# jp-schneider/awesome

Measured on AMD Instinct MI355X. Metric: INR-fits/sec (256x256 grid, convexity prior), higher is better.
Workload: dtype f32; 1 GPU; 1 x 256x256 synthetic convex blob per GPU, ConvexNextNet(h=130,L=1), SE(sigmoid) mean, Adam lr 2e-3, clamp, E=2000 full-batch steps (BASELINE configs[1]); images_per_gpu=1, grid=256x256, epochs_per_fit=2000, parallelism=dp1 (independent fits)

## Files before the change

awesome_amd/csrc/icnn_step2.h:

```cpp
#pragma once
#include "icnn_step.h"


namespace {

template <int H, int C>
struct Cfg2 {
    using G1 = Cfg<H, C>;
    static constexpr int TM = G1::TM, HM = G1::HM, HR = G1::HR, NEXT = G1::NEXT, NRL = G1::NRL, KG = G1::KG, PT = G1::PT;
    static constexpr int S = G1::S, SA = G1::SA, SB = G1::SB, RPW = G1::RPW;
    static constexpr int ext_pos(int e) { return G1::ext_pos(e); }
    static constexpr int nr_in(int tk) { return G1::nr_in(tk); }
    static constexpr int OFF_SC = 0;
    static constexpr int OFF_WINE = OFF_SC + 8;
    static constexpr int OFF_WIN = OFF_WINE + 4 * PT;
    static constexpr int OFF_BIN = OFF_WIN + C * 16;
    static constexpr int OFF_FLOOR = OFF_BIN + 16;
    static constexpr int OFF_WO = OFF_FLOOR + 16;
    static constexpr int OFF_WCT0 = OFF_WO + PT;
    static constexpr int OFF_WCT1 = OFF_WCT0 + HR * PT;
    static constexpr int WREG = round_up(H * S + 16, 256);
    static constexpr int OFF_W0 = round_up(OFF_WCT1 + HR * PT, 4);
    static constexpr int OFF_W1 = OFF_W0 + WREG;
    static constexpr int IMG_FLOATS = OFF_W1 + WREG;
    static constexpr int STAGE_FLOATS = SP * SA + 16 + SP * SB + 16;
    static constexpr bool ALIAS = STAGE_FLOATS <= WREG;
    static constexpr int OFF_STA = ALIAS ? OFF_W1 : IMG_FLOATS;
    static constexpr int OFF_STB = OFF_STA + SP * SA + 16;
    static constexpr int OFF_ACC = ALIAS ? IMG_FLOATS : IMG_FLOATS + STAGE_FLOATS;
    static constexpr int LDS_FLOATS = OFF_ACC + 4 * PT;
    static constexpr int LDS_BYTES = LDS_FLOATS * 4;
    static_assert(LDS_BYTES <= 160 * 1024, "LDS budget exceeded");
    static_assert(OFF_W0 % 4 == 0 && IMG_FLOATS % 4 == 0, "alignment");
    static constexpr int P_WIN = 0;
    static constexpr int P_BIN = H * C;
    static constexpr int P_W1 = P_BIN + H;
    static constexpr int P_B1 = P_W1 + H * H;
// ... 52 lines not shown
        constexpr int NV4 = G::IMG_FLOATS / 4;
        for (int i0 = 0; i0 < NV4; i0 += 8 * WG_THREADS) {
            f32x4 tmp[8];
#pragma unroll
            for (int k = 0; k < 8; ++k) {
                const int i = i0 + tid + k * WG_THREADS;
                if (i < NV4) tmp[k] = src[i];
            }
#pragma unroll
            for (int k = 0; k < 8; ++k) {
                const int i = i0 + tid + k * WG_THREADS;
                if (i < NV4) ((f32x4*)smem)[i] = tmp[k];
            }
        }
    }
    float cfg_ = 0.f, cbg_ = 0.f;
    if (TRAIN) {
        cfg_ = a.coef[2 * img];
        cbg_ = a.coef[2 * img + 1];
        for (int i = tid; i < 4 * PT; i += WG_THREADS) accW[i] = 0.f;
    }
    __syncthreads();
    const float b_o = smem[G::OFF_SC];
    float s_o[C];
#pragma unroll
    for (int c = 0; c < C; ++c) s_o[c] = smem[G::OFF_SC + 1 + c];
    float wol[HRA];
#pragma unroll
    for (int u = 0; u < HRA; ++u) wol[u] = HR > 0 ? woT[HM + u] : 0.f;
    const bool row_ok = wave * RPW < TM;
    const int arow = 16 * wave * RPW + l15;

    f32x4 dWa[RPW][KG], dWb[RPW][KG];
    f32x4 dL0[TM];
    float dwol[HRA], dWla[HRA][KG], dWlb[HRA][KG], dL0l[HRA][NEXT];
    float loss_acc = 0.f, dbo = 0.f, dso[C];
    if (TRAIN) {
#pragma unroll
        for (int j = 0; j < RPW; ++j)
#pragma unroll
            for (int b = 0; b < KG; ++b) {
                dWa[j][b] = f32x4{0.f, 0.f, 0.f, 0.f};
                dWb[j][b] = f32x4{0.f, 0.f, 0.f, 0.f};
            }
#pragma unroll
        for (int t = 0; t < TM; ++t) dL0[t] = f32x4{0.f, 0.f, 0.f, 0.f};
#pragma unroll
        for (int u = 0; u < HRA; ++u) {
            dwol[u] = 0.f;
#pragma unroll
            for (int b = 0; b < KG; ++b) {
                dWla[u][b] = 0.f;
                dWlb[u][b] = 0.f;
            }
#pragma unroll
            for (int e = 0; e < NEXT; ++e) dL0l[u][e] = 0.f;
        }
#pragma unroll
        for (int c = 0; c < C; ++c) dso[c] = 0.f;
    }

    auto gemm_fwd = [&](const float* Wl, const f32x4 (&B)[KG], f32x4 (&acc)[TM], float (&la)[HRA]) {
        const float* const wf = Wl + l15 * S + 4 * g;
#pragma unroll
        for (int u = 0; u < HRA; ++u) la[u] = 0.f;
        f32x4 wq[2][TM], wlq[2][HRA];
#pragma unroll
        for (int t = 0; t < TM; ++t) wq[0][t] = *(const f32x4*)(wf + t * 16 * S);
#pragma unroll
        for (int u = 0; u < HR; ++u) wlq[0][u] = *(const f32x4*)(Wl + (HM + u) * S + 4 * g);
#pragma unroll
        for (int tk = 0; tk < KG; ++tk) {
            const int cur = tk & 1, nx = cur ^ 1;
            auto next_read = [&](int i) {
                if (tk + 1 < KG) {
                    if (i < TM) wq[nx][i] = *(const f32x4*)(wf + i * 16 * S + 16 * (tk + 1));
                    else wlq[nx][i - TM] = *(const f32x4*)(Wl + (HM + i - TM) * S + 16 * (tk + 1) + 4 * g);
                }
            };
            constexpr int NRD = TM + HR;
            const int nmf = G::nr_in(tk) * TM;
            const int every = nmf / NRD > 0 ? nmf / NRD : 1;
#pragma unroll
            for (int r = 0; r < G::nr_in(tk); ++r) {
#pragma unroll
                for (int t = 0; t < TM; ++t) {
                    acc[t] = MFMA16(wq[cur][t][r], B[tk][r], (tk == 0 && r == 0) ? (f32x4{0.f, 0.f, 0.f, 0.f}) : acc[t]);
                    const int q = r * TM + t;
                    if (q % every == every - 1 && q / every < NRD) next_read(q / every);
                    OPERAND_FENCE();
                }
            }
#pragma unroll
            for (int i = 0; i < NRD; ++i)
                if (i >= nmf / every) next_read(i);
#pragma unroll
            for (int u = 0; u < HR; ++u)
#pragma unroll
                for (int r = 0; r < G::nr_in(tk); ++r) la[u] = fmaf(wlq[cur][u][r], B[tk][r], la[u]);
            __builtin_amdgcn_sched_barrier(0);
        }
    };
    auto gemm_bwd = [&](auto swap_tag, const float* Wl, const float* WcTl, const f32x4 (&dz)[TM], const float (&dzl)[HRA],
                        f32x4 (&out)[TM], float (&outl)[HRA], f32x4& outx) {
        constexpr bool SWAP = decltype(swap_tag)::value;
        float bqx[2] = {0.f, 0.f};
        outx = f32x4{0.f, 0.f, 0.f, 0.f};
        constexpr int KS = 4 * TM + HR;
        const float* const wb = Wl + l15;
#pragma unroll
        for (int u = 0; u < HRA; ++u) outl[u] = 0.f;
        float bq[2][TM];
        f32x4 wcq[2][HRA];
        auto b_row = [&](int ks) -> const float* {
            const int tk = ks >> 2, r = ks & 3;
            if (tk < TM) return wb + (16 * tk + 4 * g + r) * S;
            return wb + (g == 0 ? (HM + r) * S : 0);
        };
        {
            const float* br = b_row(0);
#pragma unroll
            for (int t = 0; t < TM; ++t) bq[0][t] = br[16 * t];
            if (DX) bqx[0] = br[16 * TM];
#pragma unroll
            for (int u = 0; u < HR; ++u) wcq[0][u] = *(const f32x4*)(WcTl + u * PT + 4 * g);
        }
#pragma unroll
        for (int ks = 0; ks < KS; ++ks) {
            const int tk = ks >> 2, r = ks & 3;
            if (ks + 1 < KS) {
                const float* br = b_row(ks + 1);
                if (DX) bqx[(ks + 1) & 1] = br[16 * TM];
            }
            if (r == 0 && (tk + 1) * 4 < KS) {
#pragma unroll
                for (int u = 0; u < HR; ++u) wcq[(tk + 1) & 1][u] = *(const f32x4*)(WcTl + u * PT + 16 * (tk + 1) + 4 * g);
            }
            OPERAND_FENCE();
            const float bop = tk < TM ? dz[tk < TM ? tk : 0][r] : (g == 0 ? dzl[r < HRA ? r : 0] : 0.f);
#pragma unroll
            for (int t = 0; t < TM; ++t) {
                const f32x4 c0 = ks == 0 ? (f32x4{0.f, 0.f, 0.f, 0.f}) : out[t];
                out[t] = SWAP ? MFMA16(bop, bq[ks & 1][t], c0) : MFMA16(bq[ks & 1][t], bop, c0);
                if (ks + 1 < KS) bq[(ks + 1) & 1][t] = b_row(ks + 1)[16 * t];
                OPERAND_FENCE();
            }
            if (DX) outx = SWAP ? MFMA16(bop, bqx[ks & 1], outx) : MFMA16(bqx[ks & 1], bop, outx);
            MFMA_STEP_FENCE();
#pragma unroll
            for (int u = 0; u < HR; ++u) {
                if (tk < TM) outl[u] = fmaf(wcq[tk & 1][u][r], dz[tk < TM ? tk : 0][r], outl[u]);
                else if (g == 0) outl[u] = fmaf(wcq[tk & 1][u][r], dzl[r < HRA ? r : 0], outl[u]);
            }
        }
    };
    const int pl = wave * 16 + l15;
    float* const sa = stA + pl * G::SA + 4 * g;
    float* const sb = stB + pl * G::SB + 4 * g;
    auto stage = [&](const f32x4 (&dz)[TM], const float (&dzl)[HRA], const f32x4 (&zp)[KG]) {
#pragma unroll
        for (int t = 0; t < TM; ++t) {
            *(f32x4*)(sa + 16 * t) = dz[t];
            *(f32x4*)(sb + 16 * t) = zp[t];
        }
        if (HR > 0 && g == 0) {
            f32x4 v = f32x4{0.f, 0.f, 0.f, 0.f};
#pragma unroll
            for (int u = 0; u < HR; ++u) v[u] = dzl[u];
            *(f32x4*)(sa + HM) = v;
        }
        if (g < 3) *(f32x4*)(sb + HM) = zp[TM];
    };
    auto dw_phase = [&](f32x4 (&dW)[RPW][KG], float (&dWl)[HRA][KG]) {
        auto stage_pt = [&](int it) { const int s = (it + wave) & 15; return 16 * (s >> 2) + (s & 3) + 4 * g; };
        float af[2][RPW], bf[2][KG];
        {
            const int pt = stage_pt(0);
#pragma unroll
            for (int j = 0; j < RPW; ++j) af[0][j] = stA[pt * G::SA + arow + 16 * j];
#pragma unroll
            for (int b = 0; b < KG; ++b) bf[0][b] = stB[pt * G::SB + 16 * b + l15];
        }
#pragma unroll
        for (int it = 0; it < SP / 4; ++it) {
            const int ptc = stage_pt(it);
// ... 210 lines not shown
            for (int t = 0; t < TM; ++t)
#pragma unroll
                for (int r = 0; r < 4; ++r) dz1[t][r] = z1[t][r] > 0.f ? dz1[t][r] : 0.f;
#pragma unroll
            for (int u = 0; u < HR; ++u) {
                const float d = sum_over_groups(dz1l[u]);
                dz1l[u] = z1l[u] > 0.f ? d : 0.f;
            }
            STAMP(4);
            __syncthreads();
            STAMP(5);
            stage(acc2, dz2l, z1);
            STAMP(6);
            {
                f32x4 dz0[TM];
                float dz0l[HRA];
                f32x4 dzx1;
                gemm_bwd(std::true_type{}, W0, smem + G::OFF_WCT0, dz1, dz1l, dz0, dz0l, dzx1);
                float wie[TM];
#pragma unroll
                for (int t = 0; t < TM; ++t) wie[t] = WinE[g * PT + 16 * t + l15];
                OPERAND_FENCE();
                f32x4 z0p[TM];
#pragma unroll
                for (int t = 0; t < TM; ++t) z0p[t] = MFMA16(xe, wie[t], (f32x4{0.f, 0.f, 0.f, 0.f}));
                MFMA_STEP_FENCE();
#pragma unroll
                for (int t = 0; t < TM; ++t)
#pragma unroll
                    for (int r = 0; r < 4; ++r) {
                        if constexpr (ACT0 == INR_ACT_RELU) dz0[t][r] = z0p[t][r] > 0.f ? dz0[t][r] : 0.f;
                        else dz0[t][r] *= dact0_f<ACT0>(z0p[t][r], a.act_omega);
                    }
                float bfe[4];
#pragma unroll
                for (int r = 0; r < 4; ++r) {
                    const int src_lane = 4 * g + r;
                    float v = 0.f;
                    if (l15 == G::ext_pos(0) - HM) v = 1.f;
#pragma unroll
                    for (int c = 0; c < C; ++c) {
                        const float xc = __shfl(x[c], src_lane);
                        if (l15 == G::ext_pos(1 + c) - HM) v = xc;
                    }
                    bfe[r] = v;
                }
#pragma unroll
                for (int r = 0; r < 4; ++r) {
#pragma unroll
                    for (int t = 0; t < TM; ++t) dL0[t] = MFMA16(dz0[t][r], bfe[r], dL0[t]);
                    MFMA_STEP_FENCE();
                }
                float hx[C];
#pragma unroll
                for (int c = 0; c < C; ++c) {
                    hx[c] = s_o[c] * dy;
                    if (DX) {
                        constexpr int dummy = 0;
                        (void)dummy;
                        const int slot = G::ext_pos(1 + c) - HM;
                        hx[c] += sum_over_groups(g == (slot >> 2) ? dzx2[slot & 3] : 0.f);
                    }
                }
#pragma unroll
                for (int u = 0; u < HR; ++u) {
                    const float d = sum_over_groups(dz0l[u]);
                    const float z0u = DX ? __shfl(z0last[u], l15) : z0last[u];
                    float dm;
                    if constexpr (ACT0 == INR_ACT_RELU) dm = z0u > 0.f ? d : 0.f;
                    else dm = d * dact0_f<ACT0>(z0lpre[u], a.act_omega);
                    if (DX) {
#pragma unroll
                        for (int c = 0; c < C; ++c) hx[c] = fmaf(WinT[c * 16 + u], dm, hx[c]);
                    }
                    if (g == 0) {
                        dL0l[u][0] += dm;
#pragma unroll
                        for (int c = 0; c < C; ++c) dL0l[u][1 + c] = fmaf(dm, x[c], dL0l[u][1 + c]);
                    }
                }
                if (DX) {
                    float part[4][C];
#pragma unroll
                    for (int r = 0; r < 4; ++r)
// ... 89 lines not shown
        constexpr int SC_DWO = 0;
        constexpr int SC_DWLA = SC_DWO + PT;
        constexpr int SC_DWLB = SC_DWLA + HRA * PT;
        constexpr int SC_L0L = SC_DWLB + HRA * PT;
        constexpr int SC_SC = SC_L0L + HRA * 4;
        constexpr int SC_L0 = SC_SC + 8;
        constexpr int WSTR = SC_L0 + HM * 4;
        static_assert(4 * WSTR <= SP * G::SA + SP * G::SB, "reduction scratch must fit the stage");
        float* const scr = stA + wave * WSTR;
#pragma unroll
        for (int t = 0; t < TM; ++t)
#pragma unroll
            for (int r = 0; r < 4; ++r)
                if (l15 == 0) scr[SC_DWO + 16 * t + 4 * g + r] = accW[wave * PT + 16 * t + 4 * g + r];
#pragma unroll
        for (int u = 0; u < HR; ++u) {
            const float v = sum_over_points(dwol[u]);
            if (lane == 0) scr[SC_DWO + HM + u] = v;
#pragma unroll
            for (int b = 0; b < KG; ++b) {
                const float wa = sum_over_groups(dWla[u][b]);
                const float wbv = sum_over_groups(dWlb[u][b]);
                if (g == 0) {
                    scr[SC_DWLA + u * PT + 16 * b + l15] = wa;
                    scr[SC_DWLB + u * PT + 16 * b + l15] = wbv;
                }
            }
#pragma unroll
            for (int e = 0; e < NEXT; ++e) {
                const float w = sum_over_points(dL0l[u][e]);
                if (lane == 0) scr[SC_L0L + u * 4 + e] = w;
            }
        }
        {
            int e = -1;
#pragma unroll
            for (int k = 0; k < NEXT; ++k)
                if (HM + l15 == G::ext_pos(k)) e = k;
            if (e >= 0) {
#pragma unroll
                for (int t = 0; t < TM; ++t)
#pragma unroll
                    for (int r = 0; r < 4; ++r) scr[SC_L0 + (16 * t + 4 * g + r) * 4 + e] = dL0[t][r];
            }
        }
        {
            float sc[2 + C];
            sc[0] = loss_acc;
            sc[1] = dbo;
#pragma unroll
            for (int c = 0; c < C; ++c) sc[2 + c] = dso[c];
#pragma unroll
            for (int k = 0; k < 2 + C; ++k) {
                const float v = sum_over_points(sc[k]);
                if (lane == 0) scr[SC_SC + k] = v;
            }
        }
        __syncthreads();
        auto wsum = [&](int i) { return ((stA[i] + stA[WSTR + i]) + stA[2 * WSTR + i]) + stA[3 * WSTR + i]; };
        for (int i = tid; i < H; i += WG_THREADS) slab[G::SL_WO + i] = wsum(SC_DWO + i);
        for (int i = tid; i < 2 * HR * PT; i += WG_THREADS) {
            const int layer = i / (HRA * PT), q = i - layer * (HRA * PT);
            const int u = q / PT, pos = q - u * PT;
            const float v = wsum((layer ? SC_DWLB : SC_DWLA) + q);
            const int lb = layer ? G::SL_L2 : G::SL_L1;
            if (pos < H) slab[lb + u * H + pos] = v;
            else if (pos == G::ext_pos(0)) slab[lb + HR * H + u] = v;
            else {
#pragma unroll
                for (int c = 0; c < C; ++c)
                    if (pos == G::ext_pos(1 + c)) slab[lb + HR * H + HR + u * C + c] = v;
            }
        }
        for (int i = tid; i < HM * NEXT; i += WG_THREADS) {
            const int row = i / NEXT, e = i - row * NEXT;
            const float v = wsum(SC_L0 + row * 4 + e);
            if (e == 0) slab[G::SL_IN + G::P_BIN + row] = v;
            else slab[G::SL_IN + G::P_WIN + row * C + (e - 1)] = v;
// ... 20 lines not shown
```

awesome_amd/csrc/icnn_step.h:

```cpp
#pragma once
#include <hip/hip_runtime.h>
#include <stdint.h>
#include <math.h>

#include <type_traits>

#include "inrfit.h"

typedef float f32x4 __attribute__((ext_vector_type(4)));
typedef float f32x2 __attribute__((ext_vector_type(2)));

#define MFMA16(a, b, c) __builtin_amdgcn_mfma_f32_16x16x4f32((a), (b), (c), 0, 0, 0)
__device__ __forceinline__ float relu0(float x) { return __int_as_float(max(__float_as_int(x), 0)); }
constexpr float INV_2PI = 0.15915494309189535f;
__device__ __forceinline__ float hw_sin(float x) { return __builtin_amdgcn_sinf(__builtin_amdgcn_fractf(x * INV_2PI)); }
__device__ __forceinline__ float hw_cos(float x) { return __builtin_amdgcn_cosf(__builtin_amdgcn_fractf(x * INV_2PI)); }
template <int ACT>
__device__ __forceinline__ float act0_f(float pre, float omega) {
    if constexpr (ACT == INR_ACT_COS) return hw_cos(pre);
    else if constexpr (ACT == INR_ACT_SIN) return hw_sin(omega * pre);
    else return relu0(pre);
}
template <int ACT>
__device__ __forceinline__ float dact0_f(float pre, float omega) {
// ... 212 lines not shown
__device__ __forceinline__ float sum_over_points(float v) {
    v += dpp_f<0xB1>(v);
    v += dpp_f<0x4E>(v);
    v += dpp_f<0x141>(v);
    v += dpp_f<0x140>(v);
    return v;
}
__device__ __forceinline__ float sum_over_groups(float v) {
    {
        const auto r = __builtin_amdgcn_permlane16_swap(__float_as_uint(v), __float_as_uint(v), false, false);
        v = __uint_as_float(r[0]) + __uint_as_float(r[1]);
    }
    {
        const auto r = __builtin_amdgcn_permlane32_swap(__float_as_uint(v), __float_as_uint(v), false, false);
        v = __uint_as_float(r[0]) + __uint_as_float(r[1]);
    }
    return v;
}

#ifndef INR_SCHED_HINTS
#define INR_SCHED_HINTS 1
#endif
#if INR_SCHED_HINTS
#define SGB(mask, n) __builtin_amdgcn_sched_group_barrier((mask), (n), 0)
#else
#define SGB(mask, n)
#endif
#ifndef INR_BWD_B128
#define INR_BWD_B128 0
#endif
#ifndef INR_STAGE_Z0_EARLY
#define INR_STAGE_Z0_EARLY 1
#endif
#ifndef INR_SLAB_NT
#define INR_SLAB_NT 1
#endif
#ifndef INR_MFMA_ORDER
#define INR_MFMA_ORDER 1
#endif
#if INR_MFMA_ORDER
#define MFMA_STEP_FENCE() __builtin_amdgcn_sched_barrier(0x7F6)
#define OPERAND_FENCE() __builtin_amdgcn_sched_barrier(0x676)
#else
#define MFMA_STEP_FENCE()
#define OPERAND_FENCE()
#endif

#ifndef INR_STAMPS
#define INR_STAMPS 0
#endif
#if INR_STAMPS
__device__ unsigned long long g_stamps[16];
__device__ unsigned long long g_wgtimes[1024][4];
#define STAMP(k)                                                                                   \
    do {                                                                                           \
        __builtin_amdgcn_sched_barrier(0);                                                         \
        unsigned long long t_;                                                                     \
        asm volatile("s_memtime %0\n\ts_waitcnt lgkmcnt(0)" : "=s"(t_)::"memory");                 \
        __builtin_amdgcn_sched_barrier(0);                                                         \
        st_sum[k] += t_ - st_prev;                                                                 \
        st_prev = t_;                                                                              \
    } while (0)
#else
#define STAMP(k)
#endif

template <int H, int C, bool TRAIN, bool DX = false, int ACT0 = INR_ACT_RELU>
__global__ __launch_bounds__(WG_THREADS, 1) void icnn_step_kernel(const StepArgs a) {
    static_assert(!DX || TRAIN, "coordinate gradients are a by-product of the backward pass");
    static_assert(!DX || ACT0 == INR_ACT_RELU, "the coordinate-gradient kernels are built for relu networks only");
    using G = Cfg<H, C>;
    constexpr int TM = G::TM, KG = G::KG, HM = G::HM, HR = G::HR, S = G::S, PT = G::PT, RPW = G::RPW, NEXT = G::NEXT;
    constexpr bool B128 = INR_BWD_B128 && (TM % 4 == 0);
    auto bcol = [](int t, int l) { return B128 ? 64 * (t >> 2) + 4 * l + (t & 3) : 16 * t + l; };
    constexpr int HRA = HR > 0 ? HR : 1;
    static_assert(TM % RPW == 0, "row tiles must split evenly over the waves that own rows");
    extern __shared__ __attribute__((aligned(16))) float smem[];
    float* const Wimg = smem + G::OFF_W;
    float* const WcT = smem + G::OFF_WCT;
    float* const WinE = smem + G::OFF_WINE;
    float* const WinT = smem + G::OFF_WIN;
    float* const binT = smem + G::OFF_BIN;
    float* const floorT = smem + G::OFF_FLOOR;
    float* const woT = smem + G::OFF_WO;
    float* const stA = smem + G::OFF_STA;
    float* const stB = smem + G::OFF_STB;

#if INR_STAMPS
    const unsigned long long rt_entry = __builtin_amdgcn_s_memrealtime();
#endif
    const int tid = threadIdx.x;
    const int lane = tid & 63;
    const int wave = __builtin_amdgcn_readfirstlane(tid >> 6);
    const int l15 = lane & 15, g = lane >> 4;
    const int img = blockIdx.x / a.wgs;
    const int wg = blockIdx.x - img * a.wgs;
    const long long N = a.N;

    {
        const f32x4* __restrict__ src = (const f32x4*)(a.wimg + (size_t)img * G::IMG_FLOATS);
        constexpr int NV4 = G::IMG_FLOATS / 4;
        constexpr int NIT = (NV4 + WG_THREADS - 1) / WG_THREADS;
        f32x4 tmp[NIT];
#pragma unroll
        for (int k = 0; k < NIT; ++k) {
            const int i = tid + k * WG_THREADS;
            if (i < NV4) tmp[k] = src[i];
        }
#pragma unroll
        for (int k = 0; k < NIT; ++k) {
            const int i = tid + k * WG_THREADS;
            if (i < NV4) ((f32x4*)smem)[i] = tmp[k];
        }
    }
    float cfg_ = 0.f, cbg_ = 0.f;
    if (TRAIN) {
        cfg_ = a.coef[2 * img];
        cbg_ = a.coef[2 * img + 1];
    }
    __syncthreads();
    const float b_o = smem[G::OFF_SC];
    float s_o[C];
#pragma unroll
    for (int c = 0; c < C; ++c) s_o[c] = smem[G::OFF_SC + 1 + c];
    float wol[HRA];
#pragma unroll
    for (int u = 0; u < HRA; ++u) wol[u] = HR > 0 ? woT[HM + u] : 0.f;

    const float* const wf = Wimg + l15 * S + 4 * g;
    const float* const wb = Wimg + l15;
    const bool row_ok = (4 * RPW == TM) || wave * RPW < TM;
    const int arow = 16 * wave * RPW + l15;

    f32x4 dW[RPW][KG];
    constexpr int NQ = (TM + 3) / 4;
    float dL0[NQ][NEXT];
    f32x4 dwo[TM];
    float dwol[HRA];
    float dWl[HRA][KG];
    float dL0l[HRA][NEXT];
    float loss_acc = 0.f, dbo = 0.f, dso[C];
    if (TRAIN) {
#pragma unroll
        for (int j = 0; j < RPW; ++j)
#pragma unroll
            for (int b = 0; b < KG; ++b) dW[j][b] = f32x4{0.f, 0.f, 0.f, 0.f};
#pragma unroll
        for (int t = 0; t < TM; ++t) dwo[t] = f32x4{0.f, 0.f, 0.f, 0.f};
#pragma unroll
        for (int q = 0; q < NQ; ++q)
#pragma unroll
            for (int e = 0; e < NEXT; ++e) dL0[q][e] = 0.f;
#pragma unroll
        for (int u = 0; u < HRA; ++u) {
            dwol[u] = 0.f;
#pragma unroll
            for (int b = 0; b < KG; ++b) dWl[u][b] = 0.f;
#pragma unroll
            for (int e = 0; e < NEXT; ++e) dL0l[u][e] = 0.f;
        }
// ... 10 lines not shown
    const float inv_width = a.grid.mode == INR_GRID_SEPARABLE ? 1.f / (float)a.grid.width : 0.f;
    auto load_point = [&](int chunk) -> PointIn {
        PointIn q;
        int pc = chunk * SP + wave * 16 + l15;
        pc = pc < (int)N ? pc : (int)N - 1;
        if (a.grid.mode == INR_GRID_SEPARABLE) {
            int row, col;
            if (fast_div) {
                row = (int)((float)pc * inv_width);
                col = pc - row * a.grid.width;
                if (col < 0) {
                    row -= 1;
                    col += a.grid.width;
                } else if (col >= a.grid.width) {
                    row += 1;
                    col -= a.grid.width;
                }
            } else {
                row = pc / a.grid.width;
                col = pc - row * a.grid.width;
            }
            q.x[0] = a.grid.xs[col];
            q.x[1] = a.grid.ys[row];
            if (C > 2) q.x[C - 1] = a.grid.ts ? a.grid.ts[img] : 0.f;
        } else {
            const float* cp = a.grid.coords + (size_t)img * a.grid.coords_image_stride;
#pragma unroll
            for (int c = 0; c < C; ++c) q.x[c] = cp[(size_t)c * N + pc];
        }
        q.tg = TRAIN ? a.targets[(size_t)img * a.data_count + min(pc, a.data_count - 1)] : 0.f;
        return q;
    };
    PointIn nxt = load_point(wg);
#if INR_STAMPS
    unsigned long long st_sum[12] = {0, 0, 0, 0, 0, 0, 0, 0, 0, 0, 0, 0}, st_prev;
    asm volatile("s_memtime %0\n\ts_waitcnt lgkmcnt(0)" : "=s"(st_prev)::"memory");
    const unsigned long long st_begin = st_prev;
    unsigned long long st_f0 = 0, st_fsum = 0;
    const unsigned long long rt_loop = __builtin_amdgcn_s_memrealtime();
#endif
    for (int chunk = wg; chunk < n_chunks; chunk += a.wgs) {
        STAMP(0);
        const int p = chunk * SP + wave * 16 + l15;
        const bool valid = p < (int)N;
        const PointIn cur = nxt;
        float x[C];
#pragma unroll
        for (int c = 0; c < C; ++c) x[c] = cur.x[c];
        const float tg = cur.tg;

        f32x4 z0[KG];
        const float xe = g < C ? x[g < C ? g : 0] : (g == C ? 1.f : 0.f);
        auto z0_tile = [&](int tk) -> f32x4 {
            f32x4 z = MFMA16(WinE[g * PT + 16 * tk + l15], xe, (f32x4{0.f, 0.f, 0.f, 0.f}));
#pragma unroll
            for (int r = 0; r < 4; ++r) z[r] = act0_f<ACT0>(z[r], a.act_omega);
            return z;
        };
        f32x4 z0lpre;
        {
            const int q = 4 * g;
            f32x4 v = *(const f32x4*)&binT[q];
#pragma unroll
            for (int c = 0; c < C; ++c) v += *(const f32x4*)&WinT[c * 16 + q] * x[c];
            const f32x4 fl = *(const f32x4*)&floorT[q];
            z0lpre = v;
#pragma unroll
            for (int r = 0; r < 4; ++r) {
                if constexpr (ACT0 == INR_ACT_RELU) {
                    z0[TM][r] = fmaxf(v[r], fl[r]);
                } else {
                    const bool hid = g == 0 && r < HR;
                    z0[TM][r] = hid ? act0_f<ACT0>(v[r], a.act_omega) : (fl[r] < 0.f ? v[r] : 0.f);
                }
// ... 537 lines not shown
```

awesome_amd/csrc/inrfit.hip:

```cpp
#include "icnn_step.h"
#include "icnn_step2.h"
#include "flow.h"
#include "rnvp.h"
#include "joint_loss.h"
#include "wide.h"
#include "star.h"
#include "cnnseg.h"
#include "fcseg.h"

#include <type_traits>
#include <vector>

namespace {

constexpr int UPD_RANGES = WIDE_MAX_LAYERS + 1;
struct UpdArgs {
    float* wimg;
    ImgMap img;
    float* params;
    float* opt_state;
    const float* slabs;
    const float* loss_part;
    long long loss_stride;
    float* loss_hist;
// ... 19 lines not shown
    const int H = m.H, C = m.C;
    if (h == H) return j;
    if (j < m.p_bin) {
        const int i = j / C;
        return i < h ? j : -1;
    }
    if (j < m.p_w[0]) {
        const int i = j - m.p_bin;
        return i < h ? h * C + i : -1;
    }
    int base_u = h * C + h;
    const int per_u = h * h + h + h * C;
    for (int k = 0; k < m.L; ++k, base_u += per_u) {
        if (j < m.p_b[k]) {
            const int q = j - m.p_w[k], o = q / H, i = q - o * H;
            return (o < h && i < h) ? base_u + o * h + i : -1;
        }
        if (j < m.p_s[k]) {
            const int o = j - m.p_b[k];
            return o < h ? base_u + h * h + o : -1;
        }
        if (j < m.p_s[k] + H * C) {
            const int q = j - m.p_s[k], o = q / C;
            return o < h ? base_u + h * h + h + q : -1;
        }
    }
    if (j < m.p_bo) {
        const int i = j - m.p_wo;
        return i < h ? base_u + i : -1;
    }
    return base_u + h + (j - m.p_bo);
}

constexpr int UPD_MAX_PARAMS = 256;
constexpr int UPD_GROUPS = 16;

constexpr int UPD_LINE = 32;

struct UpdSplit {
    int ppb;
    int n_wide;
    int blocks;
};
inline UpdSplit upd_split(int cols, int reserve = 0) {
    static const int forced = getenv("INRFIT_UPD_LINES") ? atoi(getenv("INRFIT_UPD_LINES")) : 0;
    const int cus = 256 - reserve, lines = (cols + UPD_LINE - 1) / UPD_LINE, max_lpb = UPD_MAX_PARAMS / UPD_LINE;
    int lpb = forced > 0 ? forced : (lines + cus - 1) / cus;
    if (lpb < 1) lpb = 1;
    if (lpb > max_lpb) lpb = max_lpb;
    UpdSplit sp;
    sp.ppb = lpb * UPD_LINE;
    if (forced > 0 || lpb == 1 || lines >= lpb * cus) {
        sp.blocks = (lines + lpb - 1) / lpb;
        sp.n_wide = sp.blocks;
    } else {
        sp.blocks = cus;
        sp.n_wide = lines - (lpb - 1) * cus;
    }
    return sp;
}
inline dim3 upd_grid(int cols, int n_images, int reserve = 0) { return dim3(upd_split(cols, reserve).blocks, n_images); }
inline dim3 upd_block(int cols, int reserve = 0) { return dim3(upd_split(cols, reserve).ppb / 4, UPD_GROUPS); }

#if INR_STAMPS
__device__ unsigned long long g_updtimes[512][4];
#define UPD_STAMP(k)                                                                                          \
    if (threadIdx.x == 0 && threadIdx.y == 0 && img == 0 && bx < 512) {                                       \
        __builtin_amdgcn_s_waitcnt(0);                                                                        \
        g_updtimes[bx][k] = __builtin_amdgcn_s_memrealtime();                                                 \
    }
#else
#define UPD_STAMP(k)
#endif
static_assert(UPD_GROUPS == LOSS_GROUPS, "the loss column is summed in the update's group order");
__device__ __forceinline__ void icnn_update_body(const UpdArgs& u, const int bx, const int img, const int n_wide) {
    const int tx = threadIdx.x, grp = threadIdx.y;
    const int ppbw = 4 * blockDim.x;
    const int ppb = bx < n_wide ? ppbw : ppbw - UPD_LINE;
    const int col0 = bx < n_wide ? bx * ppbw : bx * (ppbw - UPD_LINE) + n_wide * UPD_LINE;
    __shared__ float red[UPD_GROUPS][UPD_MAX_PARAMS];
    __shared__ float redl[UPD_GROUPS];
    UPD_STAMP(0);
    const int jl = grp * blockDim.x + tx;
    const int j = jl < ppb ? slab_param_of_col(u.img, col0 + jl) : -1;
    const int ju = (j >= 0 && j < u.P) ? user_param_index(u.img, u.hu, j) : -1;
    float* __restrict__ st = u.opt_state + (size_t)img * (2 * (size_t)u.Pu + INR_OPT_HEADER_FLOATS);
    float* __restrict__ hdr = st + 2 * (size_t)u.Pu;
    float p_old = 0.f, m_old = 0.f, v_old = 0.f, lr_now = 0.f;
    bool bad_before = false;
    if (u.mode == 0 && j >= 0) {
        bad_before = hdr[6 + (u.t & 1)] != 0.f;
        lr_now = hdr[u.t & 1];
        if (ju >= 0) {
            p_old = u.params[(size_t)img * u.Pu + ju];
            m_old = st[ju];
            v_old = st[u.Pu + ju];
        }
    }
    {
        const int j4 = col0 + 4 * tx;
        f32x4 part = f32x4{0.f, 0.f, 0.f, 0.f};
        if (4 * tx < ppb && j4 < u.PS && slab_param_of_col(u.img, j4) >= 0) {
            const float* __restrict__ sl = u.slabs + (size_t)img * u.wgs * u.PS + j4;
            int w = grp;
            for (; w + 15 * UPD_GROUPS < u.wgs; w += 16 * UPD_GROUPS) {
                f32x4 q[16];
#pragma unroll
                for (int k = 0; k < 16; ++k) q[k] = *(const f32x4*)(sl + (size_t)(w + k * UPD_GROUPS) * u.PS);
#pragma unroll
                for (int k = 0; k < 16; ++k) part += q[k];
            }
            for (; w < u.wgs; w += UPD_GROUPS) part += *(const f32x4*)(sl + (size_t)w * u.PS);
        }
        *(f32x4*)&red[grp][4 * tx] = part;
        if (u.mode == 0 && tx == 0) {
            redl[grp] = loss_column_group_sum(u.loss_part + (size_t)img * u.wgs * u.loss_stride, u.wgs, (size_t)u.loss_stride, grp);
        }
    }
    UPD_STAMP(1);
    __syncthreads();
    if (j < 0) return;
    float gsum = 0.f;
#pragma unroll
    for (int k = 0; k < UPD_GROUPS; ++k) gsum += red[k][jl];
    if (u.gscale != nullptr && j < u.P) gsum *= u.gscale[img];

    UPD_STAMP(2);
    if (u.mode == 1) {
        if (ju >= 0) u.grads_out[(size_t)img * u.Pu + ju] = gsum;
        else if (j == u.P) u.loss_out[img] = gsum;
        return;
    }
    float loss_now = 0.f;
#pragma unroll
    for (int k = 0; k < UPD_GROUPS; ++k) loss_now += redl[k];
    const bool frozen = bad_before || !isfinite(loss_now) || (u.gscale != nullptr && !isfinite(u.gscale[img]));
    if (j == u.P) {
        const float loss = gsum;
        if (u.loss_hist) u.loss_hist[(size_t)img * u.hist_stride + u.hist_idx] = loss;
        float lr = lr_now;
        hdr[6 + ((u.t + 1) & 1)] = frozen ? 1.f : 0.f;
        if (frozen) {
            if (u.status) u.status[img] = INR_STATUS_NONFINITE;
        } else if (u.opt.plateau) {
            float best = hdr[3];
            int num_bad = (int)hdr[4];
            if (loss < best * (1.f - u.opt.plateau_threshold)) {
                best = loss;
                num_bad = 0;
            } else {
                num_bad += 1;
            }
            if (num_bad > u.opt.plateau_patience) {
                const float nlr = fmaxf(lr * u.opt.plateau_factor, u.opt.plateau_min_lr);
                if (lr - nlr > u.opt.plateau_eps) lr = nlr;
                num_bad = 0;
            }
            hdr[3] = best;
            hdr[4] = (float)num_bad;
        }
        hdr[(u.t + 1) & 1] = lr;
        hdr[2] = lr;
        hdr[5] = loss;
        return;
    }
    if (frozen || !isfinite(gsum) || ju < 0) return;
    if (u.opt.freeze_skips) {
#pragma unroll
        for (int k = 0; k < UPD_RANGES; ++k)
            if (j >= u.freeze_lo[k] && j < u.freeze_hi[k]) return;
    }
    if (u.opt.freeze_input && j < u.input_hi) return;

    const float lr = lr_now;
    float p = p_old, m = m_old, v = v_old;
    float grad = gsum;
    if (u.opt.weight_decay != 0.f) grad = __fadd_rn(grad, __fmul_rn(u.opt.weight_decay, p));
    const double bc1 = u.bc1;
    const float w1 = u.one_minus_b1;
    m = __fadd_rn(m, __fmul_rn(w1, __fsub_rn(grad, m)));
    if (u.opt.kind == INR_OPT_ADAM) {
        const float bc2_sqrt = u.bc2_sqrt;
        const float step_size = (float)((double)lr / bc1);
        v = __fadd_rn(__fmul_rn(v, u.opt.beta2), __fmul_rn(__fmul_rn(u.one_minus_b2, grad), grad));
        const float denom = __fadd_rn(__fdiv_rn(__fsqrt_rn(v), bc2_sqrt), u.opt.eps);
        p = __fadd_rn(p, __fdiv_rn(__fmul_rn(-step_size, m), denom));
    } else {
        v = fmaxf(__fmul_rn(v, u.opt.beta2), __fadd_rn(fabsf(grad), u.opt.eps));
        const float clr = (float)((double)lr / bc1);
        p = __fadd_rn(p, __fdiv_rn(__fmul_rn(-clr, m), v));
    }
    if (u.opt.clamp) {
        bool in = false;
#pragma unroll
        for (int k = 0; k < UPD_RANGES; ++k) in = in || (j >= u.clamp_lo[k] && j < u.clamp_hi[k]);
        if (in) p = fmaxf(p, 0.f);
    }
    u.params[(size_t)img * u.Pu + ju] = p;
    if (u.wimg != nullptr) {
        int slot[2];
        const int ns = image_slots(u.img, j, slot);
        float* __restrict__ wi = u.wimg + (size_t)img * u.img.floats;
        wi[slot[0]] = p;
        if (ns > 1) wi[slot[1]] = p;
    }
    st[ju] = m;
    st[u.Pu + ju] = v;
    UPD_STAMP(3);
}

__global__ __launch_bounds__(UPD_MAX_PARAMS / 4 * UPD_GROUPS) void icnn_update_kernel(const UpdArgs u, const int n_wide) { icnn_update_body(u, blockIdx.x, blockIdx.y, n_wide); }

constexpr int UPD_UNION_MAX_THREADS = 768;
__global__ __launch_bounds__(UPD_UNION_MAX_THREADS) void cdn_update_kernel(const UpdArgs ui, const FlowUpdArgs uf, const int nbi, const int n_wide) {
    if ((int)blockIdx.x < nbi) {
        icnn_update_body(ui, blockIdx.x, blockIdx.y, n_wide);
        return;
    }
    const int tid = threadIdx.y * blockDim.x + threadIdx.x;
    if (tid >= 256) return;
    flow_update_body<32>(uf, (int)blockIdx.x - nbi, blockIdx.y, tid);
}
template <int C>
__global__ __launch_bounds__(UPD_UNION_MAX_THREADS) void pcn_update_kernel(const UpdArgs ui, const RnvpUpdArgs ur, const int nbi, const int n_wide) {
    if ((int)blockIdx.x < nbi) {
        icnn_update_body(ui, blockIdx.x, blockIdx.y, n_wide);
        return;
    }
    const int tid = threadIdx.y * blockDim.x + threadIdx.x;
    if (tid >= 256) return;
    rnvp_update_body<C>(ur, (int)blockIdx.x - nbi, blockIdx.y, tid);
}
inline bool upd_union_ok(int cols, int reserve) {
    const dim3 b = upd_block(cols, reserve);
    const int n = (int)(b.x * b.y);
    static const bool off = getenv("INRFIT_SPLIT_UPDATES") != nullptr;
    return !off && n >= 256 && n <= UPD_UNION_MAX_THREADS;
// ... 2867 lines not shown
        th[i] = fast_tanh(x[i]);
        ex[i] = fast_exp(x[i]);
    }
}

int inrfit_debug_tanh_exp(const float* x, int64_t n, float* tanh_out, float* exp_out, void* stream) {
    if (!x || !tanh_out || !exp_out || n <= 0) return INR_EINVAL;
    hipLaunchKernelGGL(debug_tanh_exp_kernel, dim3((unsigned)((n + 255) / 256)), dim3(256), 0, (hipStream_t)stream, x, (long long)n,
                       tanh_out, exp_out);
    return hipGetLastError() == hipSuccess ? INR_OK : INR_ELAUNCH;
}

int inrfit_miou(const float* out, const float* tgt, int n_images, int64_t n_points, float thr_out, float thr_tgt, int invert,
                float* iou, void* stream) {
    if (!out || !tgt || !iou || n_images <= 0 || n_points <= 0) return INR_EINVAL;
    hipLaunchKernelGGL(miou_kernel, dim3(n_images), dim3(256), 0, (hipStream_t)stream, out, tgt, (long long)n_points, thr_out,
                       thr_tgt, invert, iou);
    return hipGetLastError() == hipSuccess ? INR_OK : INR_ELAUNCH;
}

int inrfit_pack_masks(const float* values, int n_images, int64_t n_points, float threshold, int invert, uint64_t* bits,
                      void* stream) {
    if (!values || !bits || n_images <= 0 || n_points <= 0) return INR_EINVAL;
    const long long words = (n_points + 63) / 64;
    hipLaunchKernelGGL(pack_masks_kernel, dim3((unsigned)((words + 3) / 4), n_images), dim3(256), 0, (hipStream_t)stream, values,
                       (long long)n_points, threshold, invert, (unsigned long long*)bits);
    return hipGetLastError() == hipSuccess ? INR_OK : INR_ELAUNCH;
}

#if INR_STAMPS
int inrfit_debug_updtimes(unsigned long long* host_out) {
    return hipMemcpyFromSymbol(host_out, HIP_SYMBOL(g_updtimes), sizeof(unsigned long long) * 2048) == hipSuccess ? 0 : -4;
}
int inrfit_debug_stamps2(unsigned long long* host_out) {
    return hipMemcpyFromSymbol(host_out, HIP_SYMBOL(g_stamps2), sizeof(unsigned long long) * 16) == hipSuccess ? 0 : -4;
}
int inrfit_debug_stamps(unsigned long long* host_out) {
    return hipMemcpyFromSymbol(host_out, HIP_SYMBOL(g_stamps), sizeof(unsigned long long) * 16) == hipSuccess ? 0 : -4;
}
int inrfit_debug_wgtimes(unsigned long long* host_out) {
    if (hipMemcpyFromSymbol(host_out, HIP_SYMBOL(g_wgtimes), sizeof(unsigned long long) * 4096) != hipSuccess) return -4;
    static unsigned long long zeros[4096];
    return hipMemcpyToSymbol(HIP_SYMBOL(g_wgtimes), zeros, sizeof(zeros)) == hipSuccess ? 0 : -4;
}
#endif

const char* inrfit_strerror(int code) {
    switch (code) {
        case INR_OK: return "ok";
        case INR_EINVAL: return "invalid argument";
        case INR_EUNSUPPORTED: return "model shape has no compiled kernel";
        case INR_EWORKSPACE: return "workspace too small";
        case INR_ELAUNCH: return "HIP launch failed";
        case INR_ENODEVICE: return "no gfx950 device";
        default: return "unknown error";
    }
}

}


namespace {

struct FcWs {
    int P, blocks;
    long long count;
// ... 127 lines not shown
```

Before: 6.693 fits/s.

## Replace dL0 MFMA outer product with permlane transposes and scalar FMAs

The first-layer weight gradient for the input-extension columns was computed with TM MFMA ops per r against a mostly-zero broadcast operand built with shuffles. It now transposes dz0 fragments with permlane32/permlane16 swaps, broadcasts x values via readlane, and accumulates only the NEXT useful columns with scalar FMAs, shrinking dL0 accumulator registers. Separately, the backward GEMM's residual-row tail is packed into a single extra k-step by distributing the HR residual rows across lane groups instead of HR separate steps. This cuts wasted MFMA work and registers, but adds permlane and readlane traffic and changes the write-out indexing, which brings correctness risk.

```diff
diff --git a/awesome_amd/csrc/icnn_step2.h b/awesome_amd/csrc/icnn_step2.h
--- a/awesome_amd/csrc/icnn_step2.h
+++ b/awesome_amd/csrc/icnn_step2.h
@@ -3,6 +3,17 @@
 
 
 namespace {
+
+__device__ __forceinline__ void swap_halves(float& u, float& v) {
+    const auto s = __builtin_amdgcn_permlane32_swap(__float_as_uint(u), __float_as_uint(v), false, false);
+    u = __uint_as_float(s[0]);
+    v = __uint_as_float(s[1]);
+}
+__device__ __forceinline__ void swap_rows(float& u, float& v) {
+    const auto s = __builtin_amdgcn_permlane16_swap(__float_as_uint(u), __float_as_uint(v), false, false);
+    u = __uint_as_float(s[0]);
+    v = __uint_as_float(s[1]);
+}
 
 template <int H, int C>
 struct Cfg2 {
@@ -121,7 +132,8 @@
     const int arow = 16 * wave * RPW + l15;
 
     f32x4 dWa[RPW][KG], dWb[RPW][KG];
-    f32x4 dL0[TM];
+    constexpr int NQ = (TM + 3) / 4;
+    float dL0[NQ][NEXT];
     float dwol[HRA], dWla[HRA][KG], dWlb[HRA][KG], dL0l[HRA][NEXT];
     float loss_acc = 0.f, dbo = 0.f, dso[C];
     if (TRAIN) {
@@ -133,7 +145,9 @@
                 dWb[j][b] = f32x4{0.f, 0.f, 0.f, 0.f};
             }
 #pragma unroll
-        for (int t = 0; t < TM; ++t) dL0[t] = f32x4{0.f, 0.f, 0.f, 0.f};
+        for (int q = 0; q < NQ; ++q)
+#pragma unroll
+            for (int e = 0; e < NEXT; ++e) dL0[q][e] = 0.f;
 #pragma unroll
         for (int u = 0; u < HRA; ++u) {
             dwol[u] = 0.f;
@@ -195,7 +209,10 @@
         constexpr bool SWAP = decltype(swap_tag)::value;
         float bqx[2] = {0.f, 0.f};
         outx = f32x4{0.f, 0.f, 0.f, 0.f};
-        constexpr int KS = 4 * TM + HR;
+        constexpr int KS = 4 * TM + (HR > 0 ? 1 : 0);
+        float dzlg = 0.f;
+#pragma unroll
+        for (int u = 0; u < HR; ++u) dzlg = g == u ? dzl[u] : dzlg;
         const float* const wb = Wl + l15;
 #pragma unroll
         for (int u = 0; u < HRA; ++u) outl[u] = 0.f;
@@ -204,7 +221,7 @@
         auto b_row = [&](int ks) -> const float* {
             const int tk = ks >> 2, r = ks & 3;
             if (tk < TM) return wb + (16 * tk + 4 * g + r) * S;
-            return wb + (g == 0 ? (HM + r) * S : 0);
+            return wb + (g < HR ? (HM + g) * S : 0);
         };
         {
             const float* br = b_row(0);
@@ -226,7 +243,7 @@
                 for (int u = 0; u < HR; ++u) wcq[(tk + 1) & 1][u] = *(const f32x4*)(WcTl + u * PT + 16 * (tk + 1) + 4 * g);
             }
             OPERAND_FENCE();
-            const float bop = tk < TM ? dz[tk < TM ? tk : 0][r] : (g == 0 ? dzl[r < HRA ? r : 0] : 0.f);
+            const float bop = tk < TM ? dz[tk < TM ? tk : 0][r] : dzlg;
 #pragma unroll
             for (int t = 0; t < TM; ++t) {
                 const f32x4 c0 = ks == 0 ? (f32x4{0.f, 0.f, 0.f, 0.f}) : out[t];
@@ -239,7 +256,10 @@
 #pragma unroll
             for (int u = 0; u < HR; ++u) {
                 if (tk < TM) outl[u] = fmaf(wcq[tk & 1][u][r], dz[tk < TM ? tk : 0][r], outl[u]);
-                else if (g == 0) outl[u] = fmaf(wcq[tk & 1][u][r], dzl[r < HRA ? r : 0], outl[u]);
+                else if (g == 0) {
+#pragma unroll
+                    for (int v = 0; v < HR; ++v) outl[u] = fmaf(wcq[tk & 1][u][v], dzl[v], outl[u]);
+                }
             }
         }
     };
@@ -516,24 +536,31 @@
                         if constexpr (ACT0 == INR_ACT_RELU) dz0[t][r] = z0p[t][r] > 0.f ? dz0[t][r] : 0.f;
                         else dz0[t][r] *= dact0_f<ACT0>(z0p[t][r], a.act_omega);
                     }
-                float bfe[4];
 #pragma unroll
                 for (int r = 0; r < 4; ++r) {
-                    const int src_lane = 4 * g + r;
-                    float v = 0.f;
-                    if (l15 == G::ext_pos(0) - HM) v = 1.f;
-#pragma unroll
-                    for (int c = 0; c < C; ++c) {
-                        const float xc = __shfl(x[c], src_lane);
-                        if (l15 == G::ext_pos(1 + c) - HM) v = xc;
+                    float D[NQ][4];
+#pragma unroll
+                    for (int q = 0; q < NQ; ++q) {
+#pragma unroll
+                        for (int j = 0; j < 4; ++j) D[q][j] = 4 * q + j < TM ? dz0[4 * q + j < TM ? 4 * q + j : 0][r] : 0.f;
+                        swap_halves(D[q][0], D[q][2]);
+                        swap_halves(D[q][1], D[q][3]);
+                        swap_rows(D[q][0], D[q][1]);
+                        swap_rows(D[q][2], D[q][3]);
                     }
-                    bfe[r] = v;
-                }
-#pragma unroll
-                for (int r = 0; r < 4; ++r) {
-#pragma unroll
-                    for (int t = 0; t < TM; ++t) dL0[t] = MFMA16(dz0[t][r], bfe[r], dL0[t]);
-                    MFMA_STEP_FENCE();
+#pragma unroll
+                    for (int k = 0; k < 4; ++k) {
+                        float xp[C];
+#pragma unroll
+                        for (int c = 0; c < C; ++c) xp[c] = __int_as_float(__builtin_amdgcn_readlane(__float_as_int(x[c]), 4 * k + r));
+#pragma unroll
+                        for (int q = 0; q < NQ; ++q) {
+                            dL0[q][0] += D[q][k];
+#pragma unroll
+                            for (int c = 0; c < C; ++c) dL0[q][1 + c] = fmaf(D[q][k], xp[c], dL0[q][1 + c]);
+                        }
+                    }
+                    __builtin_amdgcn_sched_barrier(0);
                 }
                 float hx[C];
 #pragma unroll
@@ -689,18 +716,12 @@
                 if (lane == 0) scr[SC_L0L + u * 4 + e] = w;
             }
         }
-        {
-            int e = -1;
-#pragma unroll
-            for (int k = 0; k < NEXT; ++k)
-                if (HM + l15 == G::ext_pos(k)) e = k;
-            if (e >= 0) {
-#pragma unroll
-                for (int t = 0; t < TM; ++t)
-#pragma unroll
-                    for (int r = 0; r < 4; ++r) scr[SC_L0 + (16 * t + 4 * g + r) * 4 + e] = dL0[t][r];
-            }
-        }
+#pragma unroll
+        for (int q = 0; q < NQ; ++q)
+            if (4 * q + g < TM) {
+#pragma unroll
+                for (int e = 0; e < NEXT; ++e) scr[SC_L0 + (16 * (4 * q + g) + l15) * 4 + e] = dL0[q][e];
+            }
         {
             float sc[2 + C];
             sc[0] = loss_acc;
```

Result: no change. 6.692 fits/s (-0.0%).

## Issue prologue weight-image and update slab loads early to hide latency

Applied to the files above, without the earlier changes.

The step kernel now copies the weight image into LDS with asynchronous global_load_lds and defers the barrier and scalar reads until after the first point is loaded, so global latency overlaps other prologue work. The update kernel issues its first batch of slab loads before reading optimizer state and precomputes the clamp, freeze and image-slot decisions and the step size ahead of the reduction barrier. Both changes shorten the serial prologue and epilogue latency of the small per-step kernels. They add register pressure (16 float4 held across the state loads) and depend on the direct-to-LDS load path. Timing-stamp probes are also added under the stamps flag.

```diff
diff --git a/awesome_amd/csrc/icnn_step.h b/awesome_amd/csrc/icnn_step.h
--- a/awesome_amd/csrc/icnn_step.h
+++ b/awesome_amd/csrc/icnn_step.h
@@ -268,6 +268,9 @@
 #ifndef INR_STAGE_Z0_EARLY
 #define INR_STAGE_Z0_EARLY 1
 #endif
+#ifndef INR_PROLOGUE_EARLY
+#define INR_PROLOGUE_EARLY 1
+#endif
 #ifndef INR_SLAB_NT
 #define INR_SLAB_NT 1
 #endif
@@ -288,6 +291,7 @@
 #if INR_STAMPS
 __device__ unsigned long long g_stamps[16];
 __device__ unsigned long long g_wgtimes[1024][4];
+__device__ unsigned long long g_wgfirst[1024];
 #define STAMP(k)                                                                                   \
     do {                                                                                           \
         __builtin_amdgcn_sched_barrier(0);                                                         \
@@ -300,6 +304,27 @@
 #else
 #define STAMP(k)
 #endif
+
+template <int FLOATS>
+__device__ __forceinline__ f32x4 image_to_lds_issue(const float* __restrict__ gimg, float* smem, const int tid, const int lane, const int wave) {
+    constexpr int PIECES = FLOATS / 256, TAIL4 = (FLOATS - 256 * PIECES) / 4;
+    static_assert(FLOATS % 4 == 0 && TAIL4 <= 256, "the tail is one float4 per thread at most");
+    f32x4 tail = f32x4{0.f, 0.f, 0.f, 0.f};
+    if (tid < TAIL4) tail = ((const f32x4*)gimg)[64 * PIECES + tid];
+#pragma unroll
+    for (int k = 0; k < (PIECES + 3) / 4; ++k) {
+        const int pc = wave + 4 * k;
+        if (pc < PIECES)
+            __builtin_amdgcn_global_load_lds((const __attribute__((address_space(1))) void*)(gimg + pc * 256 + lane * 4),
+                                             (__attribute__((address_space(3))) void*)(smem + pc * 256), 16, 0, 0);
+    }
+    return tail;
+}
+template <int FLOATS>
+__device__ __forceinline__ void image_tail_to_lds(float* smem, const int tid, const f32x4 tail) {
+    constexpr int PIECES = FLOATS / 256, TAIL4 = (FLOATS - 256 * PIECES) / 4;
+    if (tid < TAIL4) ((f32x4*)smem)[64 * PIECES + tid] = tail;
+}
 
 template <int H, int C, bool TRAIN, bool DX = false, int ACT0 = INR_ACT_RELU>
 __global__ __launch_bounds__(WG_THREADS, 1) void icnn_step_kernel(const StepArgs a) {
@@ -333,8 +358,14 @@
     const int wg = blockIdx.x - img * a.wgs;
     const long long N = a.N;
 
+    const float* __restrict__ gimg = a.wimg + (size_t)img * G::IMG_FLOATS;
+#if INR_PROLOGUE_EARLY
+    static_assert(WG_THREADS == 256, "image_to_lds_issue");
+    const f32x4 img_tail = image_to_lds_issue<G::IMG_FLOATS>(gimg, smem, tid, lane, wave);
+    __builtin_amdgcn_sched_barrier(0);
+#else
     {
-        const f32x4* __restrict__ src = (const f32x4*)(a.wimg + (size_t)img * G::IMG_FLOATS);
+        const f32x4* __restrict__ src = (const f32x4*)gimg;
         constexpr int NV4 = G::IMG_FLOATS / 4;
         constexpr int NIT = (NV4 + WG_THREADS - 1) / WG_THREADS;
         f32x4 tmp[NIT];
@@ -349,19 +380,25 @@
             if (i < NV4) ((f32x4*)smem)[i] = tmp[k];
         }
     }
+#endif
     float cfg_ = 0.f, cbg_ = 0.f;
     if (TRAIN) {
         cfg_ = a.coef[2 * img];
         cbg_ = a.coef[2 * img + 1];
     }
-    __syncthreads();
-    const float b_o = smem[G::OFF_SC];
-    float s_o[C];
-#pragma unroll
-    for (int c = 0; c < C; ++c) s_o[c] = smem[G::OFF_SC + 1 + c];
+    float b_o, s_o[C];
     float wol[HRA];
-#pragma unroll
-    for (int u = 0; u < HRA; ++u) wol[u] = HR > 0 ? woT[HM + u] : 0.f;
+    auto image_arrived = [&]() {
+        __syncthreads();
+        b_o = smem[G::OFF_SC];
+#pragma unroll
+        for (int c = 0; c < C; ++c) s_o[c] = smem[G::OFF_SC + 1 + c];
+#pragma unroll
+        for (int u = 0; u < HRA; ++u) wol[u] = HR > 0 ? woT[HM + u] : 0.f;
+    };
+#if !INR_PROLOGUE_EARLY
+    image_arrived();
+#endif
 
     const float* const wf = Wimg + l15 * S + 4 * g;
     const float* const wb = Wimg + l15;
@@ -438,6 +475,12 @@
         return q;
     };
     PointIn nxt = load_point(wg);
+#if INR_PROLOGUE_EARLY
+    __builtin_amdgcn_sched_barrier(0);
+    image_tail_to_lds<G::IMG_FLOATS>(smem, tid, img_tail);
+    image_arrived();
+    __builtin_amdgcn_sched_barrier(0);
+#endif
 #if INR_STAMPS
     unsigned long long st_sum[12] = {0, 0, 0, 0, 0, 0, 0, 0, 0, 0, 0, 0}, st_prev;
     asm volatile("s_memtime %0\n\ts_waitcnt lgkmcnt(0)" : "=s"(st_prev)::"memory");
@@ -446,6 +489,14 @@
     const unsigned long long rt_loop = __builtin_amdgcn_s_memrealtime();
 #endif
     for (int chunk = wg; chunk < n_chunks; chunk += a.wgs) {
+#if INR_STAMPS
+        if (chunk == wg) {
+            __builtin_amdgcn_sched_barrier(0);
+            __builtin_amdgcn_s_waitcnt(0);
+            if (tid == 0 && blockIdx.x < 1024) g_wgfirst[blockIdx.x] = __builtin_amdgcn_s_memrealtime() - rt_entry;
+            __builtin_amdgcn_sched_barrier(0);
+        }
+#endif
         STAMP(0);
         const int p = chunk * SP + wave * 16 + l15;
         const bool valid = p < (int)N;
diff --git a/awesome_amd/csrc/inrfit.hip b/awesome_amd/csrc/inrfit.hip
--- a/awesome_amd/csrc/inrfit.hip
+++ b/awesome_amd/csrc/inrfit.hip
@@ -75,6 +75,9 @@
     return base_u + h + (j - m.p_bo);
 }
 
+#ifndef INR_UPD_SLABS_FIRST
+#define INR_UPD_SLABS_FIRST 1
+#endif
 constexpr int UPD_MAX_PARAMS = 256;
 constexpr int UPD_GROUPS = 16;
 
@@ -107,6 +110,9 @@
 
 #if INR_STAMPS
 __device__ unsigned long long g_updtimes[512][4];
+__device__ unsigned long long g_updissue[512];
+#define UPD_STAMP_ISSUE()                                                                                     \
+    if (threadIdx.x == 0 && threadIdx.y == 0 && img == 0 && bx < 512) g_updissue[bx] = __builtin_amdgcn_s_memrealtime()
 #define UPD_STAMP(k)                                                                                          \
     if (threadIdx.x == 0 && threadIdx.y == 0 && img == 0 && bx < 512) {                                       \
         __builtin_amdgcn_s_waitcnt(0);                                                                        \
@@ -114,6 +120,7 @@
     }
 #else
 #define UPD_STAMP(k)
+#define UPD_STAMP_ISSUE()
 #endif
 static_assert(UPD_GROUPS == LOSS_GROUPS, "the loss column is summed in the update's group order");
 __device__ __forceinline__ void icnn_update_body(const UpdArgs& u, const int bx, const int img, const int n_wide) {
@@ -125,33 +132,72 @@
     __shared__ float redl[UPD_GROUPS];
     UPD_STAMP(0);
     const int jl = grp * blockDim.x + tx;
-    const int j = jl < ppb ? slab_param_of_col(u.img, col0 + jl) : -1;
-    const int ju = (j >= 0 && j < u.P) ? user_param_index(u.img, u.hu, j) : -1;
+    const int j4 = col0 + 4 * tx;
+    const bool takes = 4 * tx < ppb && j4 < u.PS;
+    const float* __restrict__ sl = u.slabs + (size_t)img * u.wgs * u.PS + j4;
+    const bool trip = takes && grp + 15 * UPD_GROUPS < u.wgs;
+    f32x4 q[16];
+    auto request_slabs = [&]() {
+        UPD_STAMP_ISSUE();
+        if (trip) {
+#pragma unroll
+            for (int k = 0; k < 16; ++k) q[k] = *(const f32x4*)(sl + (size_t)(grp + k * UPD_GROUPS) * u.PS);
+        }
+        __builtin_amdgcn_sched_barrier(0);
+    };
+#if INR_UPD_SLABS_FIRST
+    request_slabs();
+#endif
     float* __restrict__ st = u.opt_state + (size_t)img * (2 * (size_t)u.Pu + INR_OPT_HEADER_FLOATS);
     float* __restrict__ hdr = st + 2 * (size_t)u.Pu;
     float p_old = 0.f, m_old = 0.f, v_old = 0.f, lr_now = 0.f;
     bool bad_before = false;
-    if (u.mode == 0 && j >= 0) {
+    if (u.mode == 0 && jl < ppb) {
         bad_before = hdr[6 + (u.t & 1)] != 0.f;
         lr_now = hdr[u.t & 1];
-        if (ju >= 0) {
-            p_old = u.params[(size_t)img * u.Pu + ju];
-            m_old = st[ju];
-            v_old = st[u.Pu + ju];
+    }
+    __builtin_amdgcn_sched_barrier(0);
+    const int j = jl < ppb ? slab_param_of_col(u.img, col0 + jl) : -1;
+    const int ju = (j >= 0 && j < u.P) ? user_param_index(u.img, u.hu, j) : -1;
+    if (u.mode == 0 && ju >= 0) {
+        p_old = u.params[(size_t)img * u.Pu + ju];
+        m_old = st[ju];
+        v_old = st[u.Pu + ju];
+    }
+#if !INR_UPD_SLABS_FIRST
+    __builtin_amdgcn_sched_barrier(0);
+    request_slabs();
+#endif
+    int slot[2] = {0, 0}, n_slots = 0;
+    bool never_updated = false, clamped = false;
+    if (u.mode == 0 && ju >= 0) {
+        if (u.wimg != nullptr) n_slots = image_slots(u.img, j, slot);
+        if (u.opt.freeze_skips) {
+#pragma unroll
+            for (int k = 0; k < UPD_RANGES; ++k) never_updated = never_updated || (j >= u.freeze_lo[k] && j < u.freeze_hi[k]);
         }
-    }
+        if (u.opt.freeze_input && j < u.input_hi) never_updated = true;
+        if (u.opt.clamp) {
+#pragma unroll
+            for (int k = 0; k < UPD_RANGES; ++k) clamped = clamped || (j >= u.clamp_lo[k] && j < u.clamp_hi[k]);
+        }
+    }
+    __builtin_amdgcn_sched_barrier(0);
     {
-        const int j4 = col0 + 4 * tx;
         f32x4 part = f32x4{0.f, 0.f, 0.f, 0.f};
-        if (4 * tx < ppb && j4 < u.PS && slab_param_of_col(u.img, j4) >= 0) {
-            const float* __restrict__ sl = u.slabs + (size_t)img * u.wgs * u.PS + j4;
+        if (takes) {
             int w = grp;
-            for (; w + 15 * UPD_GROUPS < u.wgs; w += 16 * UPD_GROUPS) {
-                f32x4 q[16];
-#pragma unroll
-                for (int k = 0; k < 16; ++k) q[k] = *(const f32x4*)(sl + (size_t)(w + k * UPD_GROUPS) * u.PS);
+            if (trip) {
 #pragma unroll
                 for (int k = 0; k < 16; ++k) part += q[k];
+                w += 16 * UPD_GROUPS;
+            }
+            for (; w + 15 * UPD_GROUPS < u.wgs; w += 16 * UPD_GROUPS) {
+                f32x4 r[16];
+#pragma unroll
+                for (int k = 0; k < 16; ++k) r[k] = *(const f32x4*)(sl + (size_t)(w + k * UPD_GROUPS) * u.PS);
+#pragma unroll
+                for (int k = 0; k < 16; ++k) part += r[k];
             }
             for (; w < u.wgs; w += UPD_GROUPS) part += *(const f32x4*)(sl + (size_t)w * u.PS);
         }
@@ -160,6 +206,8 @@
             redl[grp] = loss_column_group_sum(u.loss_part + (size_t)img * u.wgs * u.loss_stride, u.wgs, (size_t)u.loss_stride, grp);
         }
     }
+    float step_size = 0.f;
+    if (ju >= 0) step_size = (float)((double)lr_now / u.bc1);
     UPD_STAMP(1);
     __syncthreads();
     if (j < 0) return;
@@ -207,45 +255,28 @@
         hdr[5] = loss;
         return;
     }
-    if (frozen || !isfinite(gsum) || ju < 0) return;
-    if (u.opt.freeze_skips) {
-#pragma unroll
-        for (int k = 0; k < UPD_RANGES; ++k)
-            if (j >= u.freeze_lo[k] && j < u.freeze_hi[k]) return;
-    }
-    if (u.opt.freeze_input && j < u.input_hi) return;
-
-    const float lr = lr_now;
+    if (frozen || !isfinite(gsum) || ju < 0 || never_updated) return;
+
     float p = p_old, m = m_old, v = v_old;
     float grad = gsum;
     if (u.opt.weight_decay != 0.f) grad = __fadd_rn(grad, __fmul_rn(u.opt.weight_decay, p));
-    const double bc1 = u.bc1;
     const float w1 = u.one_minus_b1;
     m = __fadd_rn(m, __fmul_rn(w1, __fsub_rn(grad, m)));
     if (u.opt.kind == INR_OPT_ADAM) {
         const float bc2_sqrt = u.bc2_sqrt;
-        const float step_size = (float)((double)lr / bc1);
         v = __fadd_rn(__fmul_rn(v, u.opt.beta2), __fmul_rn(__fmul_rn(u.one_minus_b2, grad), grad));
         const float denom = __fadd_rn(__fdiv_rn(__fsqrt_rn(v), bc2_sqrt), u.opt.eps);
         p = __fadd_rn(p, __fdiv_rn(__fmul_rn(-step_size, m), denom));
     } else {
         v = fmaxf(__fmul_rn(v, u.opt.beta2), __fadd_rn(fabsf(grad), u.opt.eps));
-        const float clr = (float)((double)lr / bc1);
-        p = __fadd_rn(p, __fdiv_rn(__fmul_rn(-clr, m), v));
-    }
-    if (u.opt.clamp) {
-        bool in = false;
-#pragma unroll
-        for (int k = 0; k < UPD_RANGES; ++k) in = in || (j >= u.clamp_lo[k] && j < u.clamp_hi[k]);
-        if (in) p = fmaxf(p, 0.f);
-    }
+        p = __fadd_rn(p, __fdiv_rn(__fmul_rn(-step_size, m), v));
+    }
+    if (clamped) p = fmaxf(p, 0.f);
     u.params[(size_t)img * u.Pu + ju] = p;
-    if (u.wimg != nullptr) {
-        int slot[2];
-        const int ns = image_slots(u.img, j, slot);
+    if (n_slots > 0) {
         float* __restrict__ wi = u.wimg + (size_t)img * u.img.floats;
         wi[slot[0]] = p;
-        if (ns > 1) wi[slot[1]] = p;
+        if (n_slots > 1) wi[slot[1]] = p;
     }
     st[ju] = m;
     st[u.Pu + ju] = v;
@@ -3179,6 +3210,12 @@
 int inrfit_debug_updtimes(unsigned long long* host_out) {
     return hipMemcpyFromSymbol(host_out, HIP_SYMBOL(g_updtimes), sizeof(unsigned long long) * 2048) == hipSuccess ? 0 : -4;
 }
+int inrfit_debug_updissue(unsigned long long* host_out) {
+    return hipMemcpyFromSymbol(host_out, HIP_SYMBOL(g_updissue), sizeof(unsigned long long) * 512) == hipSuccess ? 0 : -4;
+}
+int inrfit_debug_wgfirst(unsigned long long* host_out) {
+    return hipMemcpyFromSymbol(host_out, HIP_SYMBOL(g_wgfirst), sizeof(unsigned long long) * 1024) == hipSuccess ? 0 : -4;
+}
 int inrfit_debug_stamps2(unsigned long long* host_out) {
     return hipMemcpyFromSymbol(host_out, HIP_SYMBOL(g_stamps2), sizeof(unsigned long long) * 16) == hipSuccess ? 0 : -4;
 }
```

Measured after the change: 6.691 fits/s before, 6.840 fits/s after (median of 6 runs). 2.2% higher.
